# jkomijani/normflow_

Hardware: NVIDIA B200
Metric: samples/sec (flow fwd+logJ+action) 64^2 phi^4 (higher is better)
Workload: dtype f32

## Files before the change

normflow__b200/csrc/nfk_fused_tc.cu:

```cuda

#include <stdlib.h>

#include <type_traits>

#include "nfk_common.cuh"
#include "nfk_fused_tc.cuh"

using namespace nfk;

struct TcArgs {
    const float *x, *w1, *b1, *w2, *b2, *w3, *b3, *log_in;
    float *y, *log_out;
    long long B;
    TcGeom g;
    RqsCfg cfg;
    long long* trace;
    float *save_h1, *save_h2;
    float *save_out;
};

static long long* g_trace = nullptr;
extern "C" void nfk_debug_tc_trace(long long* device_buffer) { g_trace = device_buffer; }

namespace {

// ... 15 lines not shown
    lo = make_uint4(tc_pack(l[0], l[1]), tc_pack(l[2], l[3]), tc_pack(l[4], l[5]), tc_pack(l[6], l[7]));
}

template <int KIND, int K, int INV, bool SAVE>
__global__ void __launch_bounds__(kTcThreads, 2) fused2d_tc_kernel(const TcArgs a) {
    constexpr int P = KIND == 0 ? 2 : 3 * K - 2;
    using Shape = TcShape<P>;
    constexpr int N3 = Shape::N3;
    extern __shared__ __align__(128) uint8_t smem[];
    const TcGeom& g = a.g;
    const int tid = threadIdx.x, warp = tid >> 5, lane = tid & 31;
    const int WS = g.WS, L0 = g.L0, L1 = g.L1;

    float* xs = reinterpret_cast<float*>(smem + g.off_xs);
    uint8_t* h1 = smem + g.off_h1 + kTcGuard * 16;
    uint8_t* h2 = smem + g.off_h2 + kTcGuard * 16;
    __half* B2 = reinterpret_cast<__half*>(smem + g.off_b2);
    __half* B3 = reinterpret_cast<__half*>(smem + g.off_b3);
    float* w1s = reinterpret_cast<float*>(smem + g.off_w1);
    float* b1s = w1s + 72;
    float* b2s = b1s + 8;
    float* b3s = b2s + 8;
    uint64_t* bars = reinterpret_cast<uint64_t*>(smem + g.off_bar);
    uint32_t* tmem_slot = reinterpret_cast<uint32_t*>(bars + 24);
    float* red = reinterpret_cast<float*>(tmem_slot + 2);

    for (int e = tid; e < 9 * 16 * 8; e += kTcThreads) {
        const int ci = e & 7, n = (e >> 3) & 15, t = e >> 7;
        const int co = n & 7;
        const float w = NFK_LDG(a.w2 + (co * 8 + ci) * 9 + t);
        const __half hi = __float2half_rn(w);
        const __half val = n < 8 ? hi : __float2half_rn((w - __half2float(hi)) * kLoScale);
        B2[((t * 2 + 0) * 16 + n) * 8 + ci] = val;
        B2[((t * 2 + 1) * 16 + n) * 8 + ci] = val;
    }
    for (int e = tid; e < 9 * N3 * 8; e += kTcThreads) {
        const int ci = e & 7, n = (e >> 3) % N3, t = (e >> 3) / N3;
        const int grp = n >> 4, w16 = n & 15;
        const int gs = P - 8 * grp < 8 ? P - 8 * grp : 8;
        const bool is_lo = w16 >= gs;
        const int p = 8 * grp + (is_lo ? w16 - gs : w16);
        __half val = __float2half_rn(0.f);
        if (w16 < 2 * gs) {
            const float w = NFK_LDG(a.w3 + (p * 8 + ci) * 9 + t);
            const __half hi = __float2half_rn(w);
            val = is_lo ? __float2half_rn((w - __half2float(hi)) * kLoScale) : hi;
        }
        B3[((t * 2 + 0) * N3 + n) * 8 + ci] = val;
        B3[((t * 2 + 1) * N3 + n) * 8 + ci] = val;
    }
    for (int e = tid; e < 72 + 8 + 8 + P; e += kTcThreads) {
        float v;
        if (e < 72) v = kTwoLog2e * NFK_LDG(a.w1 + (e & 7) * 9 + (e >> 3));
        else if (e < 80) v = a.b1 ? kTwoLog2e * NFK_LDG(a.b1 + e - 72) : 0.f;
        else if (e < 88) v = a.b2 ? kTwoLog2e * NFK_LDG(a.b2 + e - 80) : 0.f;
        else v = (a.b3 && e - 88 < P) ? NFK_LDG(a.b3 + e - 88) : 0.f;
        w1s[e] = v;
    }
    if (tid == 0) {
        for (int i = 0; i < 24; ++i) tc::mbar_init(tc::smem_u32(bars + i), 1);
        tc::fence_mbar_init();
    }
    if (warp == kTcComputeWarps) tc::tmem_alloc(tc::smem_u32(tmem_slot), kTcTmemCols);
    tc::fence_async_smem();
    tc::fence_before_sync();
    __syncthreads();
    tc::fence_after_sync();
    const uint32_t tmem = *tmem_slot;
    const int cbase = tc_cbase(WS);

    struct Unit { long long b; int r0; };
    const int Rr = g.R;
    auto next_unit = [&](Unit u) {
        u.r0 += Rr;
        if (u.r0 >= L0) { u.r0 = 0; u.b += gridDim.x; }
        return u;
    };

    if (warp >= kTcComputeWarps) {
        const int iw = warp - kTcComputeWarps;
        const bool lead = tc::elect_one();
        const uint32_t idesc2 = tc::make_idesc(0, 128, 16), idesc3 = tc::make_idesc(0, 128, N3);
        const uint64_t a1_desc = tc::make_desc(tc::smem_u32(h1), g.h1_comp_bytes, 128);
        const uint64_t a2_desc0 = tc::make_desc(tc::smem_u32(h2), g.h2_comp_bytes, 128);
        const uint64_t a2_desc1 = tc::make_desc(tc::smem_u32(h2 + g.h2_par_bytes), g.h2_comp_bytes, 128);
        const uint64_t b2_desc = tc::make_desc(tc::smem_u32(B2), 16 * 16, 128);
        const uint64_t b3_desc = tc::make_desc(tc::smem_u32(B3), N3 * 16, 128);
        int tn = 0;
        auto stamp = [&](int) {
            if (a.trace && blockIdx.x == 0 && lead && iw == 0 && tn < 4000) a.trace[4096 + tn++] = clock64();
        };
        for (Unit u{blockIdx.x, 0}; u.b < a.B; u = next_unit(u)) {
            const int r0 = u.r0, rows = L0 - r0 < Rr ? L0 - r0 : Rr;
            const int c2 = tc_carry(r0);
            const int t2 = tc_tiles2(rows, WS, c2), t3 = tc_tiles3(rows, WS, L1);
            const int plin = (g.active_val - 1 + g.mask_parity - r0) & 1;
            stamp(0);
            tc::bar_sync(kBarH1, kTcThreads);
            tc::fence_after_sync();
            stamp(1);
            if (lead) {
                for (int j = iw; j < t2; j += kTcIssuers) {
#pragma unroll
                    for (int t = 0; t < 9; ++t) {
                        const int delta = (t / 3 - 1) * WS + (t % 3 - 1);
                        tc::mma_f16(tmem + j * 16, tc::desc_advance(a1_desc, j * 128 + (c2 + 1) * WS + delta),
                                    tc::desc_advance(b2_desc, t * 2 * 16), idesc2, t > 0);
                    }
                    tc::mma_commit(tc::smem_u32(bars + j));
                }
            }
            __syncwarp();
            stamp(2);
            tc::bar_sync(kBarH2, kTcThreads);
            tc::fence_after_sync();
            stamp(3);
            if (lead) {
                for (int k = iw; k < t3; k += kTcIssuers) {
#pragma unroll
                    for (int t = 0; t < 9; ++t) {
                        const int sh = plin + (t / 3 - 1) * WS + (t % 3 - 1);
                        const uint64_t ad = (sh & 1) ? a2_desc1 : a2_desc0;
                        tc::mma_f16(tmem + k * N3, tc::desc_advance(ad, cbase + k * 128 + (sh >> 1)),
                                    tc::desc_advance(b3_desc, t * 2 * N3), idesc3, t > 0);
                    }
                    tc::mma_commit(tc::smem_u32(bars + 16 + k));
                }
            }
            __syncwarp();
            stamp(4);
        }
    } else {
        const int q = warp & 3, set = warp >> 2;
        uint32_t ph2 = 0, ph3 = 0;
        const uint32_t lane_addr = tmem + ((uint32_t)(q * 32) << 16);
        const bool has_b3 = a.b3 != nullptr;
        const int xs_stride = (Rr + 7) * WS;

        constexpr int kXPerThread = 6;
        float xr[kXPerThread];
        auto xload_issue = [&](const Unit& u) {
            const int rows = L0 - u.r0 < Rr ? L0 - u.r0 : Rr;
            const float* xb = a.x + u.b * (long long)L0 * L1;
            const int n = (rows + 6) * WS;
#pragma unroll
            for (int k = 0; k < kXPerThread; ++k) {
                const int e = tid + k * kTcComputeThreads;
                xr[k] = 0.f;
                if (e < n) {
                    const int j = tc_div(e, g.magic_ws), slot = e - j * WS;
                    int r = u.r0 - 3 + j;
                    r += r < 0 ? L0 : 0;
                    r += r < 0 ? L0 : 0;
                    r -= r >= L0 ? L0 : 0;
                    r -= r >= L0 ? L0 : 0;
                    int c = slot - 1;
                    c = c < 0 ? c + L1 : c;
                    c = c >= L1 ? c - L1 : c;
                    xr[k] = NFK_LDG(xb + r * L1 + c);
                }
            }
        };
        auto xload_store = [&](const Unit& u, float* xbuf) {
            const int rows = L0 - u.r0 < Rr ? L0 - u.r0 : Rr;
            const int n = (rows + 6) * WS;
#pragma unroll
// ... 57 lines not shown
                for (int s = 0; s < 2; ++s) {
#pragma unroll
                    for (int co = 0; co < 8; ++co) vv[s][co] = tanh_from_scaled(acc[z][s][co]);
                    make_records(vv[s], rec[s][0], rec[s][1]);
                }
                const int c = cc[z], i1 = (2 * jp[z]) * WS + c + 1;
#pragma unroll
                for (int s = 0; s < 2; ++s) {
                    if (s == 1 && 2 * jp[z] + 1 >= rows + 4) break;
                    const bool take_active = (s == 0) == up_active[z];
                    uint4 hi, lo;
                    hi.x = take_active ? rec[0][0].x : rec[1][0].x; hi.y = take_active ? rec[0][0].y : rec[1][0].y;
                    hi.z = take_active ? rec[0][0].z : rec[1][0].z; hi.w = take_active ? rec[0][0].w : rec[1][0].w;
                    lo.x = take_active ? rec[0][1].x : rec[1][1].x; lo.y = take_active ? rec[0][1].y : rec[1][1].y;
                    lo.z = take_active ? rec[0][1].z : rec[1][1].z; lo.w = take_active ? rec[0][1].w : rec[1][1].w;
                    uint8_t* dst = h1 + (i1 + s * WS) * 16;
                    *reinterpret_cast<uint4*>(dst) = hi;
                    *reinterpret_cast<uint4*>(dst + g.h1_comp_bytes) = lo;
                    if (c == 0 || c == L1 - 1) {
                        uint8_t* dw = c == 0 ? dst + L1 * 16 : dst - L1 * 16;
                        *reinterpret_cast<uint4*>(dw) = hi;
                        *reinterpret_cast<uint4*>(dw + g.h1_comp_bytes) = lo;
                    }
                    if (SAVE) {
                        const int j1 = 2 * jp[z] + s;
                        if (j1 >= 2 && r0 - 2 + j1 < L0) {
                            float* dsth = a.save_h1 + (b * 8 * L0 + (r0 - 2 + j1)) * (long long)L1 + c;
#pragma unroll
                            for (int co = 0; co < 8; ++co)
                                dsth[(long long)co * L0 * L1] = take_active ? vv[0][co] : vv[1][co];
                        }
                    }
                }
            }
        };
        auto layer1 = [&](const Unit& u, const float* xbuf) {
            const int r0 = u.r0, rows = L0 - r0 < Rr ? L0 - r0 : Rr;
            const int npair = (rows + 5) >> 1, items = npair * L1;
            int it0 = tid + tc_carry(r0) * L1;
            for (; it0 + kTcComputeThreads < items; it0 += 2 * kTcComputeThreads)
                layer1_items(std::integral_constant<int, 2>{}, it0, u.b, r0, rows, xbuf);
            if (it0 < items) layer1_items(std::integral_constant<int, 1>{}, it0, u.b, r0, rows, xbuf);
        };

        auto tile_wait = [&](uint64_t* bar, uint32_t parity) {
            if (q == 0) tc::mbar_wait(tc::smem_u32(bar), parity);
            tc::bar_sync(kBarSet0 + set, 128);
// ... 10 lines not shown
                tile_wait(bars + j, (ph2 >> j) & 1u);
                ph2 ^= 1u << j;
                float acc[16];
                tc::tmem_ld16(lane_addr + j * 16, acc);
                tc::tmem_ld_wait();
                const int i2 = c2 * WS + j * 128 + q * 32 + lane;
                const int j2 = tc_div(i2, g.magic_ws), slot = i2 - j2 * WS;
                if (j2 < rows + 2 && slot >= 1 && slot <= L1) {
                    float v[8];
#pragma unroll
                    for (int c = 0; c < 8; ++c)
                        v[c] = tanh_from_scaled(fmaf(acc[8 + c], kTwoLog2e / kLoScale, fmaf(acc[c], kTwoLog2e, bv[c])));
                    uint4 hi, lo;
                    make_records(v, hi, lo);
                    uint8_t* dst = h2 + (i2 & 1) * g.h2_par_bytes + (i2 >> 1) * 16;
                    *reinterpret_cast<uint4*>(dst) = hi;
                    *reinterpret_cast<uint4*>(dst + g.h2_comp_bytes) = lo;
                    if (slot == 1 || slot == L1) {
                        const int iw = slot == 1 ? i2 + L1 : i2 - L1;
                        uint8_t* dw = h2 + (iw & 1) * g.h2_par_bytes + (iw >> 1) * 16;
                        *reinterpret_cast<uint4*>(dw) = hi;
                        *reinterpret_cast<uint4*>(dw + g.h2_comp_bytes) = lo;
                    }
                    if (SAVE && j2 >= 1 && u.r0 - 1 + j2 < L0) {
                        float* dsth = a.save_h2 + (u.b * 8 * L0 + (u.r0 - 1 + j2)) * (long long)L1 + slot - 1;
#pragma unroll
                        for (int c = 0; c < 8; ++c) dsth[(long long)c * L0 * L1] = v[c];
                    }
                }
            }
        };

        auto epilogue3 = [&](const Unit& u, float* xbuf, int next_cols) -> float {
            const int r0 = u.r0, rows = L0 - r0 < Rr ? L0 - r0 : Rr;
            const int t3 = tc_tiles3(rows, WS, L1);
            const int plin = (g.active_val - 1 + g.mask_parity - r0) & 1;
            float lsum = 0.f;
            bool released = next_cols == 0;
            auto release_if_clear = [&](int k_next) {
                if (!released && (k_next >= t3 || k_next * N3 >= next_cols)) {
                    tc::fence_before_sync();
                    tc::bar_arrive(kBarH1, kTcThreads);
                    released = true;
                }
            };
            release_if_clear(set);
            for (int k = set; k < t3; k += kTcSets) {
                tile_wait(bars + 16 + k, (ph3 >> k) & 1u);
                ph3 ^= 1u << k;
                float prm[P];
#pragma unroll
                for (int grp = 0; grp < Shape::kFull; ++grp) {
                    float v[16];
                    tc::tmem_ld16(lane_addr + k * N3 + grp * 16, v);
                    tc::tmem_ld_wait();
#pragma unroll
                    for (int c = 0; c < 8; ++c) prm[grp * 8 + c] = fmaf(v[8 + c], 1.f / kLoScale, v[c]);
                }
                if constexpr (Shape::kTail > 0) {
                    constexpr int kT = Shape::kTail;
                    float v[2 * kT <= 8 ? 8 : 16];
                    const uint32_t col = lane_addr + k * N3 + Shape::kFull * 16;
                    if constexpr (2 * kT <= 8) tc::tmem_ld8(col, v);
                    else tc::tmem_ld16(col, v);
                    tc::tmem_ld_wait();
#pragma unroll
                    for (int c = 0; c < kT; ++c) prm[Shape::kFull * 8 + c] = fmaf(v[kT + c], 1.f / kLoScale, v[c]);
                }
                if (has_b3) {
#pragma unroll
                    for (int c = 0; c < P; ++c) prm[c] += b3s[c];
                }
                const int s = 2 * (cbase + k * 128 + q * 32 + lane) + plin;
                const int j2 = tc_div(s, g.magic_ws), slot = s - j2 * WS;
                if (j2 >= 1 && j2 <= rows && slot >= 1 && slot <= L1) {
                    if (SAVE) {
                        float* dsto = a.save_out + (u.b * P * L0 + (r0 + j2 - 1)) * (long long)L1 + slot - 1;
#pragma unroll
                        for (int c = 0; c < P; ++c) dsto[(long long)c * L0 * L1] = prm[c];
                    }
                    float* px = xbuf + (j2 + 2) * WS + slot;
                    const float xv = *px;
                    float out, l;
                    if (KIND == 0) {
                        const float t = prm[0], sc = fabsf(prm[1]);
                        if (!INV) { out = fmaf(xv, fast_ex2(-sc * kInvLn2), t); l = -sc; }
                        else { out = (xv - t) * fast_ex2(sc * kInvLn2); l = sc; }
                    } else {
                        tc_rqs<K, INV, P>(prm, a.cfg, xv, out, l);
                    }
                    *px = out;
                    lsum += l;
                }
                release_if_clear(k + kTcSets);
            }
            return lsum;
        };

        auto carry_h1 = [&](int rows) {
// ... 1 lines not shown
            for (int e = tid; e < 2 * n; e += kTcComputeThreads) {
                const int plane = e >= n, i = e - plane * n;
                uint8_t* dst = h1 + plane * g.h1_comp_bytes + (2 * WS + i) * 16;
                *reinterpret_cast<uint4*>(dst) = *reinterpret_cast<const uint4*>(dst + rows * WS * 16);
            }
        };
        auto carry_h2 = [&](int rows) {
            const int n = 2 * WS;
            for (int e = tid; e < 2 * n; e += kTcComputeThreads) {
                const int plane = e >= n, i = e - plane * n, is = rows * WS + i;
                uint8_t* h2c = h2 + plane * g.h2_comp_bytes;
                *reinterpret_cast<uint4*>(h2c + (i & 1) * g.h2_par_bytes + (i >> 1) * 16) =
                    *reinterpret_cast<const uint4*>(h2c + (is & 1) * g.h2_par_bytes + (is >> 1) * 16);
            }
        };

        Unit cur{blockIdx.x, 0};
        int buf = 0;
        float lacc = 0.f;
        int tn = 0;
        auto stamp = [&](int) {
            if (a.trace && blockIdx.x == 0 && tid == 0 && tn < 4000) a.trace[tn++] = clock64();
        };
        if (cur.b < a.B) {
            xload_issue(cur);
            xload_store(cur, xs);
            tc::bar_sync(kBarCompute, kTcComputeThreads);
            layer1(cur, xs);
            tc::fence_before_sync();
            tc::fence_async_smem();
            tc::bar_arrive(kBarH1, kTcThreads);
        }
        while (cur.b < a.B) {
            const Unit nxt = next_unit(cur);
            const bool has_next = nxt.b < a.B;
            const bool carry = has_next && tc_carry(nxt.r0) > 0;
            const int rows = L0 - cur.r0 < Rr ? L0 - cur.r0 : Rr;
            float* xcur = xs + buf * xs_stride;
            float* xnext = xs + (buf ^ 1) * xs_stride;
            stamp(0);
            if (has_next) xload_issue(nxt);
            epilogue2(cur);
            stamp(1);
            tc::fence_before_sync();
            tc::fence_async_smem();
            tc::bar_arrive(kBarH2, kTcThreads);
            if (has_next) xload_store(nxt, xnext);
            tc::bar_sync(kBarCompute, kTcComputeThreads);
            stamp(2);
            int next_cols = 0;
            if (carry) {
                carry_h1(rows);
                tc::bar_sync(kBarCompute, kTcComputeThreads);
            }
            if (has_next) {
                layer1(nxt, xnext);
                tc::fence_async_smem();
                const int nrows = L0 - nxt.r0 < Rr ? L0 - nxt.r0 : Rr;
                next_cols = 16 * tc_tiles2(nrows, WS, tc_carry(nxt.r0));
            }
            stamp(3);
            lacc += epilogue3(cur, xcur, next_cols);
            stamp(4);
            tc::bar_sync(kBarCompute, kTcComputeThreads);
            if (carry) carry_h2(rows);
            {
                float* yb = a.y + cur.b * (long long)L0 * L1;
                for (int j = warp; j < rows; j += kTcComputeWarps) {
                    const float* src = xcur + (j + 3) * WS + 1;
                    float* dst = yb + (cur.r0 + j) * L1;
                    for (int col = lane; col < L1; col += 32) dst[col] = src[col];
                }
            }
            if (cur.r0 + Rr >= L0) {
                lacc = warp_sum(lacc);
                if (lane == 0) red[warp] = lacc;
                tc::bar_sync(kBarCompute, kTcComputeThreads);
                if (tid == 0 && a.log_out) {
                    float tot = 0.f;
#pragma unroll
                    for (int w = 0; w < kTcComputeWarps; ++w) tot += red[w];
                    a.log_out[cur.b] = (a.log_in ? a.log_in[cur.b] : 0.f) + tot;
                }
                lacc = 0.f;
            }
            tc::bar_sync(kBarCompute, kTcComputeThreads);
            stamp(5);
            cur = nxt;
            buf ^= 1;
        }
    }
    tc::fence_before_sync();
    __syncthreads();
    if (warp == kTcComputeWarps) tc::tmem_dealloc(tmem, kTcTmemCols);
}

template <int KIND, int K, int INV, bool SAVE>
int tc_launch(TcArgs a, cudaStream_t st) {
    constexpr int P = KIND == 0 ? 2 : 3 * K - 2;
    struct Props { int sm_count, max_smem; };
    static const Props props = [] {
        Props p{0, 0};
        int dev = 0;
        cudaGetDevice(&dev);
        cudaDeviceGetAttribute(&p.sm_count, cudaDevAttrMultiProcessorCount, dev);
        cudaDeviceGetAttribute(&p.max_smem, cudaDevAttrMaxSharedMemoryPerBlockOptin, dev);
        if (p.sm_count <= 0) p.sm_count = 148;
        return p;
    }();
    const int sm_count = props.sm_count, max_smem = props.max_smem;
    const uint32_t budget = (uint32_t)((max_smem > 0 ? max_smem : 227 * 1024) + 1024) / 2 - 1024;
    int best = 0;
    float best_cost = 1e30f;
    TcGeom g = a.g;
    for (int R = 2; R <= a.g.L0; ++R) {
        if (!tc_plan<P>(g, R, budget)) continue;
        const float c = tc_cost_per_row<P>(g.L0, g.L1, g.WS, R);
        if (c < best_cost) { best_cost = c; best = R; }
    }
    if (const char* e = getenv("NFK_TC_R")) {
        const int r = atoi(e);
        TcGeom t = a.g;
        if (r >= 2 && r <= a.g.L0 && tc_plan<P>(t, r, budget)) best = r;
    }
    if (best == 0) return NFK_EUNSUPPORTED;
    tc_plan<P>(a.g, best, budget);
    a.g.magic_ws = (uint32_t)((0x100000000ULL + a.g.WS - 1) / a.g.WS);
    a.g.magic_l1 = (uint32_t)((0x100000000ULL + a.g.L1 - 1) / a.g.L1);
    if (ensure_dynamic_smem<fused2d_tc_kernel<KIND, K, INV, SAVE>>((int)budget) != NFK_OK) return NFK_ECUDA;
    long long grid = 2LL * sm_count;
    if (grid > a.B) grid = a.B;
    fused2d_tc_kernel<KIND, K, INV, SAVE><<<(unsigned)grid, kTcThreads, a.g.smem_bytes, st>>>(a);
    return check_launch();
}

template <int KIND, int K>
int tc_launch_dir(const TcArgs& a, int inverse, cudaStream_t st) {
    if (a.save_out) return inverse ? NFK_EINVAL : tc_launch<KIND, K, 0, true>(a, st);
    return inverse ? tc_launch<KIND, K, 1, false>(a, st) : tc_launch<KIND, K, 0, false>(a, st);
}

}

namespace nfk {

int fused2d_tc_step(const float* x, const float* w1, const float* b1, const float* w2, const float* b2,
                    const float* w3, const float* b3, int kind, const nfk_rqs_params& prm, int mask_parity,
                    int parity, int inverse, const float* log_in, float* y, float* log_out, int L0, int L1,
                    int64_t B, cudaStream_t st, float* save_h1, float* save_h2, float* save_out) {
    if ((L0 & 1) || (L1 & 1) || L1 < 2 || L0 < 2) return NFK_EUNSUPPORTED;
    if ((save_h1 || save_h2 || save_out) && !(save_h1 && save_h2 && save_out)) return NFK_EINVAL;
    TcArgs a;
    a.x = x; a.w1 = w1; a.b1 = b1; a.w2 = w2; a.b2 = b2; a.w3 = w3; a.b3 = b3;
    a.log_in = log_in; a.y = y; a.log_out = log_out; a.B = B;
    a.trace = g_trace;
// ... 20 lines not shown
```

normflow__b200/csrc/nfk_fused_tc.cuh:

```cuda
#pragma once

#include <cuda_fp16.h>

#include "nfk_fused.cuh"
#include "nfk_tc.cuh"

namespace nfk {

#ifndef NFK_TC_COMPUTE_WARPS
#define NFK_TC_COMPUTE_WARPS 8
#endif
constexpr int kTcComputeWarps = NFK_TC_COMPUTE_WARPS;
constexpr int kTcSets = kTcComputeWarps / 4;
constexpr int kTcComputeThreads = 32 * kTcComputeWarps;
#ifndef NFK_TC_ISSUERS
#define NFK_TC_ISSUERS 1
#endif
constexpr int kTcIssuers = NFK_TC_ISSUERS;
constexpr int kTcThreads = kTcComputeThreads + 32 * kTcIssuers;
constexpr int kTcTmemCols = 256;
constexpr int kTcGuard = 8;
constexpr float kLoScale = 2048.f;

enum { kBarCompute = 1, kBarH1 = 2, kBarH2 = 3, kBarSet0 = 4 };

struct TcGeom {
    int L0, L1, WS;
    int R;
    int mask_parity, active_val;
    uint32_t off_xs, off_h1, off_h2, off_b2, off_b3, off_w1, off_bar;
    uint32_t h1_comp_bytes;
    uint32_t h2_comp_bytes;
    uint32_t h2_par_bytes;
    uint32_t smem_bytes;
    uint32_t magic_ws, magic_l1;
};

__device__ __forceinline__ int tc_div(int n, uint32_t magic) { return (int)__umulhi((uint32_t)n, magic); }

NFK_HD int tc_div_up(int a, int b) { return (a + b - 1) / b; }
NFK_HD int tc_carry(int r0) { return r0 > 0 ? 2 : 0; }
NFK_HD int tc_tiles2(int rows, int WS, int carry) { return tc_div_up((rows + 2 - carry) * WS, 128); }
NFK_HD int tc_cbase(int WS) { return (WS + 1) >> 1; }
NFK_HD int tc_tiles3(int rows, int WS, int L1) {
    const int s_max = rows * WS + L1;
    return tc_div_up((s_max >> 1) - tc_cbase(WS) + 1, 128);
}
// ... 8 lines not shown
template <int P>
inline bool tc_plan(TcGeom& g, int R, uint32_t smem_budget) {
    const int WS = g.WS;
    g.R = R;
    const int t2 = tc_tiles2(R, WS, 0), t3 = tc_tiles3(R, WS, g.L1);
    if (t2 > 16 || t2 * 16 > kTcTmemCols || t3 > 8 || t3 * TcShape<P>::N3 > kTcTmemCols) return false;
    if ((R + 6) * WS > 6 * kTcComputeThreads) return false;
    auto align = [](uint32_t v) { return (v + 127u) & ~127u; };
    uint32_t off = 0;
    g.off_xs = off; off = align(off + 2u * (uint32_t)(R + 7) * WS * 4);
    const int e2 = t2 * 128 > 2 * WS + tc_tiles2(R, WS, 2) * 128 ? t2 * 128 : 2 * WS + tc_tiles2(R, WS, 2) * 128;
    const int n1 = e2 + 2 * WS + 2;
    g.h1_comp_bytes = align((uint32_t)(kTcGuard + n1) * 16);
    g.off_h1 = off; off += 2 * g.h1_comp_bytes;
    int n2 = tc_cbase(WS) + t3 * 128 + (WS + 1) / 2 + 2;
    const int n2_min = ((R + 2) * WS + 1) / 2 + 1;
    if (n2 < n2_min) n2 = n2_min;
    g.h2_comp_bytes = align((uint32_t)(kTcGuard + n2) * 16);
    g.h2_par_bytes = 2 * g.h2_comp_bytes + 64;
    g.off_h2 = off; off += 2 * g.h2_par_bytes;
    g.off_b2 = off; off = align(off + 9 * 2 * 16 * 16);
    g.off_b3 = off; off = align(off + 9 * 2 * TcShape<P>::N3 * 16);
    g.off_w1 = off; off = align(off + (72 + 8 + 8 + P) * 4);
    g.off_bar = off; off = align(off + 24 * 8 + 64);
    g.smem_bytes = off;
    return g.smem_bytes <= smem_budget;
}

template <int P>
inline float tc_cost_per_row(int L0, int L1, int WS, int R) {
    const float c2 = 9 * 41.f, c3 = 9 * (TcShape<P>::N3 <= 32 ? 42.f : TcShape<P>::N3 <= 64 ? 50.f : 66.f);
    float total = 0.f;
    for (int r0 = 0; r0 < L0; r0 += R) {
        const int rows = L0 - r0 < R ? L0 - r0 : R;
        total += tc_tiles2(rows, WS, tc_carry(r0)) * c2 + tc_tiles3(rows, WS, L1) * c3 + 600.f;
    }
    return total / L0;
}

__device__ __forceinline__ float tc_split(float v, float& lo) {
    const float hi = __uint_as_float(__float_as_uint(v) & 0xFFFFE000u);
    lo = v - hi;
    return hi;
}
__device__ __forceinline__ uint32_t tc_pack(float a, float b) {
    uint32_t r;
    asm("cvt.rn.f16x2.f32 %0, %1, %2;" : "=r"(r) : "f"(b), "f"(a));
    return r;
}

__device__ __forceinline__ float fast_ex2(float v) {
    float r;
    asm("ex2.approx.ftz.f32 %0, %1;" : "=f"(r) : "f"(v));
    return r;
// ... 103 lines not shown
```

normflow__b200/csrc/nfk_tc.cuh:

```cuda
#pragma once

#include <cuda_runtime.h>
#include <stdint.h>

namespace nfk {
namespace tc {

__device__ __forceinline__ uint32_t smem_u32(const void* p) { return (uint32_t)__cvta_generic_to_shared(p); }

__device__ __forceinline__ uint64_t make_desc(uint32_t addr, uint32_t lbo_bytes, uint32_t sbo_bytes) {
    uint64_t d = 0;
    d |= (uint64_t)((addr >> 4) & 0x3FFF);
    d |= (uint64_t)((lbo_bytes >> 4) & 0x3FFF) << 16;
    d |= (uint64_t)((sbo_bytes >> 4) & 0x3FFF) << 32;
    d |= (uint64_t)1 << 46;
    return d;
}
__device__ __forceinline__ uint64_t desc_advance(uint64_t d, int rows16) {
    return (d & ~(uint64_t)0x3FFF) | (uint64_t)(((uint32_t)(d & 0x3FFF) + (uint32_t)rows16) & 0x3FFF);
}

__host__ __device__ inline uint32_t make_idesc(int fmt, int M, int N) {
    uint32_t d = 0;
    d |= 1u << 4;
    d |= (uint32_t)fmt << 7;
    d |= (uint32_t)fmt << 10;
    d |= (uint32_t)(N >> 3) << 17;
    d |= (uint32_t)(M >> 4) << 24;
    return d;
}

__device__ __forceinline__ void mma_f16(uint32_t d_tmem, uint64_t da, uint64_t db, uint32_t idesc, uint32_t accumulate) {
    asm volatile("{\n\t.reg .pred p;\n\tsetp.ne.b32 p, %4, 0;\n\t"
                 "tcgen05.mma.cta_group::1.kind::f16 [%0], %1, %2, %3, p;\n\t}\n"
                 :: "r"(d_tmem), "l"(da), "l"(db), "r"(idesc), "r"(accumulate) : "memory");
}
__device__ __forceinline__ void mma_tf32(uint32_t d_tmem, uint64_t da, uint64_t db, uint32_t idesc, uint32_t accumulate) {
    asm volatile("{\n\t.reg .pred p;\n\tsetp.ne.b32 p, %4, 0;\n\t"
                 "tcgen05.mma.cta_group::1.kind::tf32 [%0], %1, %2, %3, p;\n\t}\n"
                 :: "r"(d_tmem), "l"(da), "l"(db), "r"(idesc), "r"(accumulate) : "memory");
}
__device__ __forceinline__ void mma_commit(uint32_t bar) {
    asm volatile("tcgen05.commit.cta_group::1.mbarrier::arrive::one.shared::cluster.b64 [%0];" :: "r"(bar) : "memory");
}

__device__ __forceinline__ void mbar_init(uint32_t bar, uint32_t count) {
    asm volatile("mbarrier.init.shared::cta.b64 [%0], %1;" :: "r"(bar), "r"(count) : "memory");
}
__device__ __forceinline__ void fence_mbar_init() { asm volatile("fence.mbarrier_init.release.cluster;" ::: "memory"); }
__device__ __forceinline__ void mbar_wait(uint32_t bar, uint32_t parity) {
    uint32_t ok = 0;
    for (int spin = 0; !ok; ++spin) {
        asm volatile("{\n\t.reg .pred p;\n\tmbarrier.try_wait.parity.shared::cta.b64 p, [%1], %2, %3;\n\t"
                     "selp.u32 %0, 1, 0, p;\n\t}\n"
                     : "=r"(ok) : "r"(bar), "r"(parity), "r"(20000u) : "memory");
        if (spin > 400000) __trap();
    }
}

__device__ __forceinline__ void mbar_arrive(uint32_t bar) {
    asm volatile("{\n\t.reg .b64 st;\n\tmbarrier.arrive.shared::cta.b64 st, [%0];\n\t}\n" :: "r"(bar) : "memory");
}

__device__ __forceinline__ void cp_async16(uint32_t dst_smem, const void* src) {
    asm volatile("cp.async.cg.shared.global [%0], [%1], 16;" :: "r"(dst_smem), "l"(src) : "memory");
}
__device__ __forceinline__ void cp_async_wait_all() { asm volatile("cp.async.wait_all;" ::: "memory"); }

__device__ __forceinline__ void tmem_alloc(uint32_t slot_smem, uint32_t cols) {
    asm volatile("tcgen05.alloc.cta_group::1.sync.aligned.shared::cta.b32 [%0], %1;" :: "r"(slot_smem), "r"(cols) : "memory");
    asm volatile("tcgen05.relinquish_alloc_permit.cta_group::1.sync.aligned;" ::: "memory");
}
__device__ __forceinline__ void tmem_dealloc(uint32_t tmem, uint32_t cols) {
    asm volatile("tcgen05.dealloc.cta_group::1.sync.aligned.b32 %0, %1;" :: "r"(tmem), "r"(cols) : "memory");
}

__device__ __forceinline__ void tmem_ld16(uint32_t taddr, float (&r)[16]) {
    uint32_t u[16];
    asm volatile("tcgen05.ld.sync.aligned.32x32b.x16.b32 {%0,%1,%2,%3,%4,%5,%6,%7,%8,%9,%10,%11,%12,%13,%14,%15}, [%16];"
                 : "=r"(u[0]), "=r"(u[1]), "=r"(u[2]), "=r"(u[3]), "=r"(u[4]), "=r"(u[5]), "=r"(u[6]), "=r"(u[7]),
                   "=r"(u[8]), "=r"(u[9]), "=r"(u[10]), "=r"(u[11]), "=r"(u[12]), "=r"(u[13]), "=r"(u[14]), "=r"(u[15])
                 : "r"(taddr));
#pragma unroll
    for (int i = 0; i < 16; ++i) r[i] = __uint_as_float(u[i]);
}
__device__ __forceinline__ void tmem_ld8(uint32_t taddr, float (&r)[8]) {
    uint32_t u[8];
    asm volatile("tcgen05.ld.sync.aligned.32x32b.x8.b32 {%0,%1,%2,%3,%4,%5,%6,%7}, [%8];"
                 : "=r"(u[0]), "=r"(u[1]), "=r"(u[2]), "=r"(u[3]), "=r"(u[4]), "=r"(u[5]), "=r"(u[6]), "=r"(u[7])
                 : "r"(taddr));
#pragma unroll
    for (int i = 0; i < 8; ++i) r[i] = __uint_as_float(u[i]);
}
__device__ __forceinline__ void tmem_ld_wait() { asm volatile("tcgen05.wait::ld.sync.aligned;" ::: "memory"); }

__device__ __forceinline__ void fence_async_smem() { asm volatile("fence.proxy.async.shared::cta;" ::: "memory"); }
__device__ __forceinline__ void fence_before_sync() { asm volatile("tcgen05.fence::before_thread_sync;" ::: "memory"); }
// ... 14 lines not shown
```

Before: 1.562 million.

## Use paired-CTA tcgen05 MMA across 2-CTA clusters with split B operands

Launches the fused kernel as 2-CTA clusters and issues tcgen05.mma with cta_group::2 (M=256) from rank 0. Each CTA holds half of the B weight matrix (hi/lo split across ranks for layer 2, half of N3 for layer 3), which halves per-CTA B staging. Named barriers become cluster mbarriers, and TMEM alloc/dealloc are paired. The multiple-issuer option is removed and an odd batch is padded with a duplicate sample whose outputs are not written. The aim is higher MMA throughput and fewer issue instructions, at the cost of cross-CTA synchronization and lockstep between the two CTAs.

```diff
diff --git a/normflow__b200/csrc/nfk_fused_tc.cu b/normflow__b200/csrc/nfk_fused_tc.cu
--- a/normflow__b200/csrc/nfk_fused_tc.cu
+++ b/normflow__b200/csrc/nfk_fused_tc.cu
@@ -1,6 +1,7 @@
 
 #include <stdlib.h>
 
+#include <algorithm>
 #include <type_traits>
 
 #include "nfk_common.cuh"
@@ -62,20 +63,22 @@
     float* b2s = b1s + 8;
     float* b3s = b2s + 8;
     uint64_t* bars = reinterpret_cast<uint64_t*>(smem + g.off_bar);
-    uint32_t* tmem_slot = reinterpret_cast<uint32_t*>(bars + 24);
+    uint32_t* tmem_slot = reinterpret_cast<uint32_t*>(bars + kTcBars);
     float* red = reinterpret_cast<float*>(tmem_slot + 2);
-
-    for (int e = tid; e < 9 * 16 * 8; e += kTcThreads) {
-        const int ci = e & 7, n = (e >> 3) & 15, t = e >> 7;
-        const int co = n & 7;
+    const uint32_t rank = tc::cluster_ctarank();
+
+    for (int e = tid; e < 9 * 8 * 8; e += kTcThreads) {
+        const int ci = e & 7, co = (e >> 3) & 7, t = e >> 6;
         const float w = NFK_LDG(a.w2 + (co * 8 + ci) * 9 + t);
         const __half hi = __float2half_rn(w);
-        const __half val = n < 8 ? hi : __float2half_rn((w - __half2float(hi)) * kLoScale);
-        B2[((t * 2 + 0) * 16 + n) * 8 + ci] = val;
-        B2[((t * 2 + 1) * 16 + n) * 8 + ci] = val;
-    }
-    for (int e = tid; e < 9 * N3 * 8; e += kTcThreads) {
-        const int ci = e & 7, n = (e >> 3) % N3, t = (e >> 3) / N3;
+        const __half val = rank == 0 ? hi : __float2half_rn((w - __half2float(hi)) * kLoScale);
+        B2[((t * 2 + 0) * 8 + co) * 8 + ci] = val;
+        B2[((t * 2 + 1) * 8 + co) * 8 + ci] = val;
+    }
+    constexpr int N3h = N3 / 2;
+    for (int e = tid; e < 9 * N3h * 8; e += kTcThreads) {
+        const int ci = e & 7, nh = (e >> 3) % N3h, t = (e >> 3) / N3h;
+        const int n = (int)rank * N3h + nh;
         const int grp = n >> 4, w16 = n & 15;
         const int gs = P - 8 * grp < 8 ? P - 8 * grp : 8;
         const bool is_lo = w16 >= gs;
@@ -86,8 +89,8 @@
             const __half hi = __float2half_rn(w);
             val = is_lo ? __float2half_rn((w - __half2float(hi)) * kLoScale) : hi;
         }
-        B3[((t * 2 + 0) * N3 + n) * 8 + ci] = val;
-        B3[((t * 2 + 1) * N3 + n) * 8 + ci] = val;
+        B3[((t * 2 + 0) * N3h + nh) * 8 + ci] = val;
+        B3[((t * 2 + 1) * N3h + nh) * 8 + ci] = val;
     }
     for (int e = tid; e < 72 + 8 + 8 + P; e += kTcThreads) {
         float v;
@@ -99,12 +102,13 @@
     }
     if (tid == 0) {
         for (int i = 0; i < 24; ++i) tc::mbar_init(tc::smem_u32(bars + i), 1);
+        for (int i = kBarH1; i < kTcBars; ++i) tc::mbar_init(tc::smem_u32(bars + i), 2 * kTcComputeWarps);
         tc::fence_mbar_init();
     }
-    if (warp == kTcComputeWarps) tc::tmem_alloc(tc::smem_u32(tmem_slot), kTcTmemCols);
+    if (warp == kTcComputeWarps) tc::tmem_alloc_pair(tc::smem_u32(tmem_slot), kTcTmemCols);
     tc::fence_async_smem();
     tc::fence_before_sync();
-    __syncthreads();
+    tc::cluster_sync();
     tc::fence_after_sync();
     const uint32_t tmem = *tmem_slot;
     const int cbase = tc_cbase(WS);
@@ -116,55 +120,57 @@
         if (u.r0 >= L0) { u.r0 = 0; u.b += gridDim.x; }
         return u;
     };
+    auto pair_live = [&](const Unit& u) { return (u.b & ~1LL) < a.B; };
 
     if (warp >= kTcComputeWarps) {
-        const int iw = warp - kTcComputeWarps;
         const bool lead = tc::elect_one();
-        const uint32_t idesc2 = tc::make_idesc(0, 128, 16), idesc3 = tc::make_idesc(0, 128, N3);
+        const uint32_t idesc2 = tc::make_idesc(0, 256, 16), idesc3 = tc::make_idesc(0, 256, N3);
         const uint64_t a1_desc = tc::make_desc(tc::smem_u32(h1), g.h1_comp_bytes, 128);
         const uint64_t a2_desc0 = tc::make_desc(tc::smem_u32(h2), g.h2_comp_bytes, 128);
         const uint64_t a2_desc1 = tc::make_desc(tc::smem_u32(h2 + g.h2_par_bytes), g.h2_comp_bytes, 128);
-        const uint64_t b2_desc = tc::make_desc(tc::smem_u32(B2), 16 * 16, 128);
-        const uint64_t b3_desc = tc::make_desc(tc::smem_u32(B3), N3 * 16, 128);
+        const uint64_t b2_desc = tc::make_desc(tc::smem_u32(B2), 8 * 16, 128);
+        const uint64_t b3_desc = tc::make_desc(tc::smem_u32(B3), N3h * 16, 128);
         int tn = 0;
         auto stamp = [&](int) {
-            if (a.trace && blockIdx.x == 0 && lead && iw == 0 && tn < 4000) a.trace[4096 + tn++] = clock64();
-        };
-        for (Unit u{blockIdx.x, 0}; u.b < a.B; u = next_unit(u)) {
+            if (a.trace && blockIdx.x == 0 && lead && tn < 4000) a.trace[4096 + tn++] = clock64();
+        };
+        uint32_t ph = 0;
+        for (Unit u{blockIdx.x, 0}; rank == 0 && pair_live(u); u = next_unit(u)) {
             const int r0 = u.r0, rows = L0 - r0 < Rr ? L0 - r0 : Rr;
             const int c2 = tc_carry(r0);
             const int t2 = tc_tiles2(rows, WS, c2), t3 = tc_tiles3(rows, WS, L1);
             const int plin = (g.active_val - 1 + g.mask_parity - r0) & 1;
             stamp(0);
-            tc::bar_sync(kBarH1, kTcThreads);
+            tc::mbar_wait_cluster(tc::smem_u32(bars + kBarH1), ph);
             tc::fence_after_sync();
             stamp(1);
             if (lead) {
-                for (int j = iw; j < t2; j += kTcIssuers) {
+                for (int j = 0; j < t2; ++j) {
 #pragma unroll
                     for (int t = 0; t < 9; ++t) {
                         const int delta = (t / 3 - 1) * WS + (t % 3 - 1);
-                        tc::mma_f16(tmem + j * 16, tc::desc_advance(a1_desc, j * 128 + (c2 + 1) * WS + delta),
-                                    tc::desc_advance(b2_desc, t * 2 * 16), idesc2, t > 0);
-                    }
-                    tc::mma_commit(tc::smem_u32(bars + j));
+                        tc::mma_f16_pair(tmem + j * 16, tc::desc_advance(a1_desc, j * 128 + (c2 + 1) * WS + delta),
+                                         tc::desc_advance(b2_desc, t * 2 * 8), idesc2, t > 0);
+                    }
+                    tc::mma_commit_pair(tc::smem_u32(bars + j));
                 }
             }
             __syncwarp();
             stamp(2);
-            tc::bar_sync(kBarH2, kTcThreads);
+            tc::mbar_wait_cluster(tc::smem_u32(bars + kBarH2), ph);
             tc::fence_after_sync();
+            ph ^= 1u;
             stamp(3);
             if (lead) {
-                for (int k = iw; k < t3; k += kTcIssuers) {
+                for (int k = 0; k < t3; ++k) {
 #pragma unroll
                     for (int t = 0; t < 9; ++t) {
                         const int sh = plin + (t / 3 - 1) * WS + (t % 3 - 1);
                         const uint64_t ad = (sh & 1) ? a2_desc1 : a2_desc0;
-                        tc::mma_f16(tmem + k * N3, tc::desc_advance(ad, cbase + k * 128 + (sh >> 1)),
-                                    tc::desc_advance(b3_desc, t * 2 * N3), idesc3, t > 0);
-                    }
-                    tc::mma_commit(tc::smem_u32(bars + 16 + k));
+                        tc::mma_f16_pair(tmem + k * N3, tc::desc_advance(ad, cbase + k * 128 + (sh >> 1)),
+                                         tc::desc_advance(b3_desc, t * 2 * N3h), idesc3, t > 0);
+                    }
+                    tc::mma_commit_pair(tc::smem_u32(bars + 16 + k));
                 }
             }
             __syncwarp();
@@ -181,7 +187,7 @@
         float xr[kXPerThread];
         auto xload_issue = [&](const Unit& u) {
             const int rows = L0 - u.r0 < Rr ? L0 - u.r0 : Rr;
-            const float* xb = a.x + u.b * (long long)L0 * L1;
+            const float* xb = a.x + (u.b < a.B ? u.b : u.b - 1) * (long long)L0 * L1;
             const int n = (rows + 6) * WS;
 #pragma unroll
             for (int k = 0; k < kXPerThread; ++k) {
@@ -285,7 +291,7 @@
                         *reinterpret_cast<uint4*>(dw) = hi;
                         *reinterpret_cast<uint4*>(dw + g.h1_comp_bytes) = lo;
                     }
-                    if (SAVE) {
+                    if (SAVE && b < a.B) {
                         const int j1 = 2 * jp[z] + s;
                         if (j1 >= 2 && r0 - 2 + j1 < L0) {
                             float* dsth = a.save_h1 + (b * 8 * L0 + (r0 - 2 + j1)) * (long long)L1 + c;
@@ -342,13 +348,20 @@
                         *reinterpret_cast<uint4*>(dw) = hi;
                         *reinterpret_cast<uint4*>(dw + g.h2_comp_bytes) = lo;
                     }
-                    if (SAVE && j2 >= 1 && u.r0 - 1 + j2 < L0) {
+                    if (SAVE && u.b < a.B && j2 >= 1 && u.r0 - 1 + j2 < L0) {
                         float* dsth = a.save_h2 + (u.b * 8 * L0 + (u.r0 - 1 + j2)) * (long long)L1 + slot - 1;
 #pragma unroll
                         for (int c = 0; c < 8; ++c) dsth[(long long)c * L0 * L1] = v[c];
                     }
                 }
             }
+        };
+
+        auto arrive_pair = [&](int bar) {
+            tc::fence_before_sync();
+            tc::fence_async_smem();
+            __syncwarp();
+            if (lane == 0) tc::mbar_arrive_cluster(tc::mapa(tc::smem_u32(bars + bar), 0));
         };
 
         auto epilogue3 = [&](const Unit& u, float* xbuf, int next_cols) -> float {
@@ -359,8 +372,7 @@
             bool released = next_cols == 0;
             auto release_if_clear = [&](int k_next) {
                 if (!released && (k_next >= t3 || k_next * N3 >= next_cols)) {
-                    tc::fence_before_sync();
-                    tc::bar_arrive(kBarH1, kTcThreads);
+                    arrive_pair(kBarH1);
                     released = true;
                 }
             };
@@ -394,7 +406,7 @@
                 const int s = 2 * (cbase + k * 128 + q * 32 + lane) + plin;
                 const int j2 = tc_div(s, g.magic_ws), slot = s - j2 * WS;
                 if (j2 >= 1 && j2 <= rows && slot >= 1 && slot <= L1) {
-                    if (SAVE) {
+                    if (SAVE && u.b < a.B) {
                         float* dsto = a.save_out + (u.b * P * L0 + (r0 + j2 - 1)) * (long long)L1 + slot - 1;
 #pragma unroll
                         for (int c = 0; c < P; ++c) dsto[(long long)c * L0 * L1] = prm[c];
@@ -442,18 +454,16 @@
         auto stamp = [&](int) {
             if (a.trace && blockIdx.x == 0 && tid == 0 && tn < 4000) a.trace[tn++] = clock64();
         };
-        if (cur.b < a.B) {
+        if (pair_live(cur)) {
             xload_issue(cur);
             xload_store(cur, xs);
             tc::bar_sync(kBarCompute, kTcComputeThreads);
             layer1(cur, xs);
-            tc::fence_before_sync();
-            tc::fence_async_smem();
-            tc::bar_arrive(kBarH1, kTcThreads);
+            arrive_pair(kBarH1);
         }
-        while (cur.b < a.B) {
+        while (pair_live(cur)) {
             const Unit nxt = next_unit(cur);
-            const bool has_next = nxt.b < a.B;
+            const bool has_next = pair_live(nxt);
             const bool carry = has_next && tc_carry(nxt.r0) > 0;
             const int rows = L0 - cur.r0 < Rr ? L0 - cur.r0 : Rr;
             float* xcur = xs + buf * xs_stride;
@@ -462,9 +472,7 @@
             if (has_next) xload_issue(nxt);
             epilogue2(cur);
             stamp(1);
-            tc::fence_before_sync();
-            tc::fence_async_smem();
-            tc::bar_arrive(kBarH2, kTcThreads);
+            arrive_pair(kBarH2);
             if (has_next) xload_store(nxt, xnext);
             tc::bar_sync(kBarCompute, kTcComputeThreads);
             stamp(2);
@@ -484,7 +492,7 @@
             stamp(4);
             tc::bar_sync(kBarCompute, kTcComputeThreads);
             if (carry) carry_h2(rows);
-            {
+            if (cur.b < a.B) {
                 float* yb = a.y + cur.b * (long long)L0 * L1;
                 for (int j = warp; j < rows; j += kTcComputeWarps) {
                     const float* src = xcur + (j + 3) * WS + 1;
@@ -496,7 +504,7 @@
                 lacc = warp_sum(lacc);
                 if (lane == 0) red[warp] = lacc;
                 tc::bar_sync(kBarCompute, kTcComputeThreads);
-                if (tid == 0 && a.log_out) {
+                if (tid == 0 && a.log_out && cur.b < a.B) {
                     float tot = 0.f;
 #pragma unroll
                     for (int w = 0; w < kTcComputeWarps; ++w) tot += red[w];
@@ -511,8 +519,10 @@
         }
     }
     tc::fence_before_sync();
-    __syncthreads();
-    if (warp == kTcComputeWarps) tc::tmem_dealloc(tmem, kTcTmemCols);
+    tc::cluster_sync();
+    tc::fence_after_sync();
+    if (warp == kTcComputeWarps) tc::tmem_dealloc_pair(tmem, kTcTmemCols);
+    tc::cluster_sync();
 }
 
 template <int KIND, int K, int INV, bool SAVE>
@@ -547,10 +557,25 @@
     tc_plan<P>(a.g, best, budget);
     a.g.magic_ws = (uint32_t)((0x100000000ULL + a.g.WS - 1) / a.g.WS);
     a.g.magic_l1 = (uint32_t)((0x100000000ULL + a.g.L1 - 1) / a.g.L1);
-    if (ensure_dynamic_smem<fused2d_tc_kernel<KIND, K, INV, SAVE>>((int)budget) != NFK_OK) return NFK_ECUDA;
-    long long grid = 2LL * sm_count;
-    if (grid > a.B) grid = a.B;
-    fused2d_tc_kernel<KIND, K, INV, SAVE><<<(unsigned)grid, kTcThreads, a.g.smem_bytes, st>>>(a);
+    constexpr auto kernel = fused2d_tc_kernel<KIND, K, INV, SAVE>;
+    if (ensure_dynamic_smem<kernel>((int)budget) != NFK_OK) return NFK_ECUDA;
+    cudaLaunchAttribute attr[1];
+    attr[0].id = cudaLaunchAttributeClusterDimension;
+    attr[0].val.clusterDim.x = 2;
+    attr[0].val.clusterDim.y = 1;
+    attr[0].val.clusterDim.z = 1;
+    cudaLaunchConfig_t cfg = {};
+    cfg.blockDim = dim3(kTcThreads);
+    cfg.stream = st;
+    cfg.attrs = attr;
+    cfg.numAttrs = 1;
+    const long long pairs = std::min<long long>(sm_count, (a.B + 1) / 2);
+    cfg.gridDim = dim3((unsigned)(2 * pairs));
+    cfg.dynamicSmemBytes = a.g.smem_bytes;
+    if (cudaLaunchKernelEx(&cfg, kernel, a) != cudaSuccess) {
+        cudaGetLastError();
+        return NFK_ECUDA;
+    }
     return check_launch();
 }
 
diff --git a/normflow__b200/csrc/nfk_fused_tc.cuh b/normflow__b200/csrc/nfk_fused_tc.cuh
--- a/normflow__b200/csrc/nfk_fused_tc.cuh
+++ b/normflow__b200/csrc/nfk_fused_tc.cuh
@@ -13,16 +13,13 @@
 constexpr int kTcComputeWarps = NFK_TC_COMPUTE_WARPS;
 constexpr int kTcSets = kTcComputeWarps / 4;
 constexpr int kTcComputeThreads = 32 * kTcComputeWarps;
-#ifndef NFK_TC_ISSUERS
-#define NFK_TC_ISSUERS 1
-#endif
-constexpr int kTcIssuers = NFK_TC_ISSUERS;
-constexpr int kTcThreads = kTcComputeThreads + 32 * kTcIssuers;
+constexpr int kTcThreads = kTcComputeThreads + 32;
 constexpr int kTcTmemCols = 256;
 constexpr int kTcGuard = 8;
 constexpr float kLoScale = 2048.f;
 
-enum { kBarCompute = 1, kBarH1 = 2, kBarH2 = 3, kBarSet0 = 4 };
+enum { kBarCompute = 1, kBarSet0 = 2 };
+constexpr int kBarH1 = 24, kBarH2 = 25, kTcBars = 26;
 
 struct TcGeom {
     int L0, L1, WS;
@@ -77,14 +74,14 @@
     g.off_b2 = off; off = align(off + 9 * 2 * 16 * 16);
     g.off_b3 = off; off = align(off + 9 * 2 * TcShape<P>::N3 * 16);
     g.off_w1 = off; off = align(off + (72 + 8 + 8 + P) * 4);
-    g.off_bar = off; off = align(off + 24 * 8 + 64);
+    g.off_bar = off; off = align(off + kTcBars * 8 + 8 + 4 * kTcComputeWarps);
     g.smem_bytes = off;
     return g.smem_bytes <= smem_budget;
 }
 
 template <int P>
 inline float tc_cost_per_row(int L0, int L1, int WS, int R) {
-    const float c2 = 9 * 41.f, c3 = 9 * (TcShape<P>::N3 <= 32 ? 42.f : TcShape<P>::N3 <= 64 ? 50.f : 66.f);
+    const float c2 = 9 * 38.5f, c3 = 9 * (TcShape<P>::N3 <= 32 ? 38.4f : 42.3f);
     float total = 0.f;
     for (int r0 = 0; r0 < L0; r0 += R) {
         const int rows = L0 - r0 < R ? L0 - r0 : R;
diff --git a/normflow__b200/csrc/nfk_tc.cuh b/normflow__b200/csrc/nfk_tc.cuh
--- a/normflow__b200/csrc/nfk_tc.cuh
+++ b/normflow__b200/csrc/nfk_tc.cuh
@@ -44,6 +44,32 @@
     asm volatile("tcgen05.commit.cta_group::1.mbarrier::arrive::one.shared::cluster.b64 [%0];" :: "r"(bar) : "memory");
 }
 
+__device__ __forceinline__ uint32_t cluster_ctarank() {
+    uint32_t r;
+    asm volatile("mov.u32 %0, %%cluster_ctarank;" : "=r"(r));
+    return r;
+}
+__device__ __forceinline__ void cluster_sync() {
+    asm volatile("barrier.cluster.arrive.release.aligned;\n\tbarrier.cluster.wait.acquire.aligned;" ::: "memory");
+}
+__device__ __forceinline__ void mma_f16_pair(uint32_t d_tmem, uint64_t da, uint64_t db, uint32_t idesc, uint32_t accumulate) {
+    asm volatile("{\n\t.reg .pred p;\n\tsetp.ne.b32 p, %4, 0;\n\t"
+                 "tcgen05.mma.cta_group::2.kind::f16 [%0], %1, %2, %3, p;\n\t}\n"
+                 :: "r"(d_tmem), "l"(da), "l"(db), "r"(idesc), "r"(accumulate) : "memory");
+}
+__device__ __forceinline__ void mma_commit_pair(uint32_t bar) {
+    asm volatile("tcgen05.commit.cta_group::2.mbarrier::arrive::one.shared::cluster.multicast::cluster.b64 [%0], %1;"
+                 :: "r"(bar), "h"((uint16_t)3) : "memory");
+}
+__device__ __forceinline__ uint32_t mapa(uint32_t addr, uint32_t rank) {
+    uint32_t r;
+    asm volatile("mapa.shared::cluster.u32 %0, %1, %2;" : "=r"(r) : "r"(addr), "r"(rank));
+    return r;
+}
+__device__ __forceinline__ void mbar_arrive_cluster(uint32_t cluster_addr) {
+    asm volatile("mbarrier.arrive.release.cluster.shared::cluster.b64 _, [%0];" :: "r"(cluster_addr) : "memory");
+}
+
 __device__ __forceinline__ void mbar_init(uint32_t bar, uint32_t count) {
     asm volatile("mbarrier.init.shared::cta.b64 [%0], %1;" :: "r"(bar), "r"(count) : "memory");
 }
@@ -52,6 +78,15 @@
     uint32_t ok = 0;
     for (int spin = 0; !ok; ++spin) {
         asm volatile("{\n\t.reg .pred p;\n\tmbarrier.try_wait.parity.shared::cta.b64 p, [%1], %2, %3;\n\t"
+                     "selp.u32 %0, 1, 0, p;\n\t}\n"
+                     : "=r"(ok) : "r"(bar), "r"(parity), "r"(20000u) : "memory");
+        if (spin > 400000) __trap();
+    }
+}
+__device__ __forceinline__ void mbar_wait_cluster(uint32_t bar, uint32_t parity) {
+    uint32_t ok = 0;
+    for (int spin = 0; !ok; ++spin) {
+        asm volatile("{\n\t.reg .pred p;\n\tmbarrier.try_wait.parity.acquire.cluster.shared::cta.b64 p, [%1], %2, %3;\n\t"
                      "selp.u32 %0, 1, 0, p;\n\t}\n"
                      : "=r"(ok) : "r"(bar), "r"(parity), "r"(20000u) : "memory");
         if (spin > 400000) __trap();
@@ -73,6 +108,13 @@
 }
 __device__ __forceinline__ void tmem_dealloc(uint32_t tmem, uint32_t cols) {
     asm volatile("tcgen05.dealloc.cta_group::1.sync.aligned.b32 %0, %1;" :: "r"(tmem), "r"(cols) : "memory");
+}
+__device__ __forceinline__ void tmem_alloc_pair(uint32_t slot_smem, uint32_t cols) {
+    asm volatile("tcgen05.alloc.cta_group::2.sync.aligned.shared::cta.b32 [%0], %1;" :: "r"(slot_smem), "r"(cols) : "memory");
+    asm volatile("tcgen05.relinquish_alloc_permit.cta_group::2.sync.aligned;" ::: "memory");
+}
+__device__ __forceinline__ void tmem_dealloc_pair(uint32_t tmem, uint32_t cols) {
+    asm volatile("tcgen05.dealloc.cta_group::2.sync.aligned.b32 %0, %1;" :: "r"(tmem), "r"(cols) : "memory");
 }
 
 __device__ __forceinline__ void tmem_ld16(uint32_t taddr, float (&r)[16]) {
diff --git a/scratch/tc_pair_probe.cu b/scratch/tc_pair_probe.cu
--- /dev/null
+++ b/scratch/tc_pair_probe.cu
@@ -0,0 +1,246 @@
+#include <cuda_fp16.h>
+#include <cuda_runtime.h>
+#include <stdint.h>
+#include <stdio.h>
+#include <stdlib.h>
+
+#include <vector>
+
+#include "../normflow__b200/csrc/nfk_fused_tc.cuh"
+
+#define CK(x) do { cudaError_t e = (x); if (e != cudaSuccess) { printf("CUDA error %s at %d\n", cudaGetErrorString(e), __LINE__); exit(1); } } while (0)
+
+using namespace nfk;
+
+constexpr int WS = 67;
+constexpr int kTiles = 8;
+constexpr int kArec = kTiles * 128 + 2 * WS + 16;
+constexpr uint32_t kPlane = kArec * 16;
+
+__device__ __forceinline__ uint32_t ctarank() {
+    uint32_t r;
+    asm volatile("mov.u32 %0, %%cluster_ctarank;" : "=r"(r));
+    return r;
+}
+__device__ __forceinline__ void cluster_sync() {
+    asm volatile("barrier.cluster.arrive.release.aligned;\n\tbarrier.cluster.wait.acquire.aligned;" ::: "memory");
+}
+template <int PAIR>
+__device__ __forceinline__ void mma(uint32_t d, uint64_t a, uint64_t b, uint32_t idesc, uint32_t acc) {
+    if (PAIR)
+        asm volatile("{\n\t.reg .pred p;\n\tsetp.ne.b32 p, %4, 0;\n\t"
+                     "tcgen05.mma.cta_group::2.kind::f16 [%0], %1, %2, %3, p;\n\t}\n"
+                     :: "r"(d), "l"(a), "l"(b), "r"(idesc), "r"(acc) : "memory");
+    else
+        tc::mma_f16(d, a, b, idesc, acc);
+}
+template <int PAIR>
+__device__ __forceinline__ void commit(uint32_t bar) {
+    if (PAIR)
+        asm volatile("tcgen05.commit.cta_group::2.mbarrier::arrive::one.shared::cluster.multicast::cluster.b64 [%0], %1;"
+                     :: "r"(bar), "h"((uint16_t)3) : "memory");
+    else
+        tc::mma_commit(bar);
+}
+template <int PAIR>
+__device__ __forceinline__ void alloc(uint32_t slot) {
+    if (PAIR) {
+        asm volatile("tcgen05.alloc.cta_group::2.sync.aligned.shared::cta.b32 [%0], 256;" :: "r"(slot) : "memory");
+        asm volatile("tcgen05.relinquish_alloc_permit.cta_group::2.sync.aligned;" ::: "memory");
+    } else {
+        tc::tmem_alloc(slot, 256);
+    }
+}
+template <int PAIR>
+__device__ __forceinline__ void dealloc(uint32_t tmem) {
+    if (PAIR) asm volatile("tcgen05.dealloc.cta_group::2.sync.aligned.b32 %0, 256;" :: "r"(tmem) : "memory");
+    else tc::tmem_dealloc(tmem, 256);
+}
+
+__host__ __device__ inline float aval(int rank, int plane, int rec, int c) {
+    const uint32_t h = (uint32_t)(((rank * 2 + plane) * 40503 + rec) * 8 + c) * 2654435761u;
+    return (float)((int)(h >> 28) % 9 - 4) * 0.125f;
+}
+__host__ __device__ inline float bval(int rank, int tap, int kg, int n, int c) {
+    const uint32_t h = (uint32_t)((((rank * 9 + tap) * 2 + kg) * 64 + n) * 8 + c) * 2246822519u;
+    return (float)((int)(h >> 28) % 9 - 4) * 0.125f;
+}
+
+template <int PAIR>
+__global__ void __launch_bounds__(kTcThreads, 2) pair_probe(int N, int reps, long long* cyc, float* chk) {
+    extern __shared__ __align__(128) uint8_t smem[];
+    __half* A = reinterpret_cast<__half*>(smem);
+    __half* Bm = reinterpret_cast<__half*>(smem + 2 * kPlane);
+    uint64_t* bar = reinterpret_cast<uint64_t*>(smem + 2 * kPlane + 9 * 2 * 64 * 16);
+    uint32_t* slot = reinterpret_cast<uint32_t*>(bar + 1);
+    const int tid = threadIdx.x, warp = tid >> 5;
+    const int rank = PAIR ? (int)ctarank() : 0;
+    const int Nb = PAIR ? N / 2 : N;
+    for (int e = tid; e < 2 * kArec * 8; e += kTcThreads)
+        A[e] = __float2half_rn(aval(rank, e / (kArec * 8), (e / 8) % kArec, e & 7));
+    for (int e = tid; e < 9 * 2 * Nb * 8; e += kTcThreads) {
+        const int c = e & 7, n = (e >> 3) % Nb, kg = (e / (8 * Nb)) & 1, t = e / (16 * Nb);
+        Bm[e] = __float2half_rn(bval(rank, t, kg, n, c));
+    }
+    if (tid == 0) { tc::mbar_init(tc::smem_u32(bar), 1); tc::fence_mbar_init(); }
+    if (warp == kTcComputeWarps) alloc<PAIR>(tc::smem_u32(slot));
+    tc::fence_async_smem();
+    tc::fence_before_sync();
+    __syncthreads();
+    cluster_sync();
+    tc::fence_after_sync();
+    const uint32_t tmem = *slot;
+    if (warp == kTcComputeWarps) {
+        const bool lead = tc::elect_one();
+        const uint32_t idesc = tc::make_idesc(0, PAIR ? 256 : 128, N);
+        const uint64_t ad = tc::make_desc(tc::smem_u32(A), kPlane, 128);
+        const uint64_t bd = tc::make_desc(tc::smem_u32(Bm), Nb * 16, 128);
+        const int slots = 256 / N;
+        long long t0 = clock64();
+        if (lead && (!PAIR || rank == 0)) {
+            if (chk) {
+                mma<PAIR>(tmem, ad, bd, idesc, 0);
+            } else {
+                for (int r = 0; r < reps; ++r)
+                    for (int j = 0; j < kTiles; ++j) {
+#pragma unroll
+                        for (int t = 0; t < 9; ++t) {
+                            const int delta = (t / 3) * WS + (t % 3);
+                            mma<PAIR>(tmem + (j % slots) * N, tc::desc_advance(ad, j * 128 + delta),
+                                      tc::desc_advance(bd, t * 2 * Nb), idesc, t > 0);
+                        }
+                    }
+            }
+            commit<PAIR>(tc::smem_u32(bar));
+        }
+        __syncwarp();
+        tc::mbar_wait(tc::smem_u32(bar), 0);
+        long long t1 = clock64();
+        if (lead) {
+            uint32_t smid;
+            asm volatile("mov.u32 %0, %%smid;" : "=r"(smid));
+            cyc[blockIdx.x] = t1 - t0;
+            cyc[2048 + blockIdx.x] = smid;
+        }
+    }
+    tc::fence_before_sync();
+    __syncthreads();
+    tc::fence_after_sync();
+    if (chk && blockIdx.x < 2 && warp < 4) {
+        const int m = warp * 32 + (tid & 31);
+        for (int c0 = 0; c0 < N; c0 += 16) {
+            float v[16];
+            tc::tmem_ld16(tmem + ((uint32_t)(warp * 32) << 16) + c0, v);
+            tc::tmem_ld_wait();
+            for (int i = 0; i < 16; ++i) chk[((size_t)rank * 128 + m) * N + c0 + i] = v[i];
+        }
+    }
+    tc::fence_before_sync();
+    __syncthreads();
+    cluster_sync();
+    if (warp == kTcComputeWarps) dealloc<PAIR>(tmem);
+}
+
+template <int PAIR>
+static void launch(int grid, int smem, int N, int reps, long long* cyc, float* chk) {
+    cudaLaunchConfig_t cfg = {};
+    cudaLaunchAttribute at[1];
+    at[0].id = cudaLaunchAttributeClusterDimension;
+    at[0].val.clusterDim.x = 2; at[0].val.clusterDim.y = 1; at[0].val.clusterDim.z = 1;
+    cfg.gridDim = dim3(grid); cfg.blockDim = dim3(kTcThreads); cfg.dynamicSmemBytes = smem;
+    cfg.attrs = at; cfg.numAttrs = 1;
+    CK(cudaLaunchKernelEx(&cfg, pair_probe<PAIR>, N, reps, cyc, chk));
+}
+
+int main() {
+    setvbuf(stdout, NULL, _IONBF, 0);
+    int dev = 0, sms = 0, max_smem = 0, clk = 0;
+    CK(cudaGetDevice(&dev));
+    CK(cudaDeviceGetAttribute(&sms, cudaDevAttrMultiProcessorCount, dev));
+    CK(cudaDeviceGetAttribute(&max_smem, cudaDevAttrMaxSharedMemoryPerBlockOptin, dev));
+    CK(cudaDeviceGetAttribute(&clk, cudaDevAttrClockRate, dev));
+    TcGeom g{};
+    g.L0 = 64; g.L1 = 64; g.WS = WS;
+    const uint32_t budget = (uint32_t)(max_smem + 1024) / 2 - 1024;
+    if (!tc_plan<28>(g, 15, budget)) { printf("plan failed\n"); return 1; }
+    const int smem = (int)g.smem_bytes;
+    printf("SMs %d, max smem/block %d, kernel smem at 64x64 P=28 R=15: %d B (budget %u), clock %d kHz\n", sms, max_smem,
+           smem, budget, clk);
+    CK(cudaFuncSetAttribute(pair_probe<0>, cudaFuncAttributeMaxDynamicSharedMemorySize, smem));
+    CK(cudaFuncSetAttribute(pair_probe<1>, cudaFuncAttributeMaxDynamicSharedMemorySize, smem));
+    cudaFuncAttributes fa;
+    CK(cudaFuncGetAttributes(&fa, pair_probe<1>));
+    printf("probe kernel: %d registers\n", fa.numRegs);
+
+    {
+        cudaLaunchConfig_t cfg = {};
+        cudaLaunchAttribute at[1];
+        at[0].id = cudaLaunchAttributeClusterDimension;
+        at[0].val.clusterDim.x = 2; at[0].val.clusterDim.y = 1; at[0].val.clusterDim.z = 1;
+        cfg.gridDim = dim3(2 * sms); cfg.blockDim = dim3(kTcThreads); cfg.dynamicSmemBytes = smem;
+        cfg.attrs = at; cfg.numAttrs = 1;
+        int ncl = 0, nblk = 0;
+        CK(cudaOccupancyMaxActiveClusters(&ncl, pair_probe<1>, &cfg));
+        CK(cudaOccupancyMaxActiveBlocksPerMultiprocessor(&nblk, pair_probe<1>, kTcThreads, smem));
+        printf("occupancy: max active clusters of 2 = %d (need %d for 2 CTAs on every SM), blocks per SM = %d\n", ncl,
+               sms, nblk);
+    }
+
+    long long* dcyc;
+    float* dchk;
+    CK(cudaMalloc(&dcyc, 4096 * 8));
+    CK(cudaMalloc(&dchk, 2 * 128 * 64 * 4));
+
+    for (int pair = 0; pair < 2; ++pair)
+        for (int N : {16, 32, 64}) {
+            CK(cudaMemset(dchk, 0, 2 * 128 * 64 * 4));
+            if (pair) launch<1>(2, smem, N, 1, dcyc, dchk); else launch<0>(2, smem, N, 1, dcyc, dchk);
+            CK(cudaDeviceSynchronize());
+            std::vector<float> h(2 * 128 * N);
+            CK(cudaMemcpy(h.data(), dchk, h.size() * 4, cudaMemcpyDeviceToHost));
+            double worst = 0;
+            for (int r = 0; r < 1 + pair; ++r)
+                for (int m = 0; m < 128; ++m)
+                    for (int n = 0; n < N; ++n) {
+                        const int br = pair ? n / (N / 2) : r, bn = pair ? n % (N / 2) : n;
+                        double ref = 0;
+                        for (int kg = 0; kg < 2; ++kg)
+                            for (int c = 0; c < 8; ++c) ref += (double)aval(r, kg, m, c) * bval(br, 0, kg, bn, c);
+                        const double d = fabs(ref - h[((size_t)r * 128 + m) * N + n]);
+                        worst = d > worst ? d : worst;
+                    }
+            printf("check %s N=%2d: max |D - ref| = %g\n", pair ? "cta_group::2 M=256" : "cta_group::1 M=128", N, worst);
+        }
+
+    const int reps = 100, nmma = reps * kTiles * 9;
+    cudaEvent_t e0, e1;
+    CK(cudaEventCreate(&e0)); CK(cudaEventCreate(&e1));
+    for (int full = 0; full < 2; ++full)
+        for (int N : {16, 32, 64})
+            for (int pair = 0; pair < 2; ++pair) {
+                const int grid = full ? 2 * sms : 2;
+                float ms = 0;
+                for (int it = 0; it < 3; ++it) {
+                    CK(cudaEventRecord(e0));
+                    if (pair) launch<1>(grid, smem, N, reps, dcyc, nullptr); else launch<0>(grid, smem, N, reps, dcyc, nullptr);
+                    CK(cudaEventRecord(e1));
+                    CK(cudaEventSynchronize(e1));
+                    CK(cudaEventElapsedTime(&ms, e0, e1));
+                }
+                std::vector<long long> h(grid), sm(grid);
+                CK(cudaMemcpy(h.data(), dcyc, grid * 8, cudaMemcpyDeviceToHost));
+                CK(cudaMemcpy(sm.data(), dcyc + 2048, grid * 8, cudaMemcpyDeviceToHost));
+                int same_sm = 0, same_tpc = 0;
+                for (int c = 0; c + 1 < grid; c += 2) { same_sm += sm[c] == sm[c + 1]; same_tpc += (sm[c] >> 1) == (sm[c + 1] >> 1); }
+                if (N == 16) printf("  placement: %d of %d clusters on one SM, %d on one SM pair (smid / 2)\n", same_sm, grid / 2, same_tpc);
+                double mean = 0, mx = 0;
+                for (long long v : h) { mean += v; mx = v > mx ? v : mx; }
+                mean /= grid;
+                const double shares = full ? 2.0 * nmma : (double)nmma;
+                printf("%s %-18s N=%2d: %d MMAs per issuer, CTA cycles mean %.0f max %.0f -> %.1f cyc per 128-row MMA per SM "
+                       "(event %.3f ms)\n", full ? "full grid" : "1 cluster", pair ? "cta_group::2 M=256" : "cta_group::1 M=128",
+                       N, nmma, mean, mx, mean / shares, ms);
+            }
+    printf("probe done\n");
+    return 0;
+}
```

Measured after the change: 1.499 million, median of 6. 0.959x the previous value.
